# falseywinchnet/PyITD

Hardware: AMD Instinct MI355X
Metric: Msamples/s full ITD (8 levels) + achieved HBM GB/s (higher is better)
Workload: dtype f64

## Files before the change

pyitd_amd/csrc/itd_engine.hip:

```cpp
#include <hip/hip_runtime.h>
#include <hip/hip_ext.h>

#include <algorithm>
#include <cstdio>
#include <cstdlib>
#include <cstring>
#include <type_traits>
#include <atomic>
#include <chrono>
#include <dlfcn.h>
#include <memory>
#include <new>
#include <thread>
#include <vector>

#include "../../include/pyitd_hip.h"
#include "itd_kernels.hpp"
#include "itd_resident.hpp"
#include "itd_knotfirst.hpp"
#include "itd_cubic.hpp"
#include "itd_detect_fast.hpp"
#include "itd_stream.hpp"
#include "itd_tfe.hpp"
#include "itd_tfe_batch.hpp"
// ... 275 lines not shown
    if (tag != ITD_TIME_DECOMPOSE && tag != ITD_TIME_KF_KNOTS) {
        if (e->span_first < 0) e->span_first = k;
        e->span_last = k;
    }
    return k;
}

constexpr int32_t kMaxGridY = 65535;
int chunk_of(const itd_engine *e, int64_t n, int32_t batch)
{
    if (e->chunk > 0) return std::min<int32_t>(std::min<int32_t>(e->chunk, kMaxGridY), batch);
    if ((int64_t)batch * n <= ((int64_t)1 << 24) && batch <= kMaxGridY) return batch;
    const int64_t per = e->batch_streams > 1 ? ((int64_t)1 << 23) : ((int64_t)1 << 24);
    const int64_t c = std::max<int64_t>(1, per / n);
    return (int)std::min<int64_t>(std::min<int64_t>(c, kMaxGridY), batch);
}

inline int64_t seq_samples(const itd_engine *e, int64_t n, int32_t batch) { return (int64_t)std::min<int32_t>(chunk_of(e, n, batch), batch) * n; }

constexpr int kKfLevels = ITD_MAX_ITERATION + 3;
int ensure_kf_ws(itd_engine *e, int tpw, bool may_allocate)
{
    const size_t wgs = (size_t)(e->max_tiles + tpw - 1) / tpw;
    if (e->d_kf && (size_t)e->kf.wgs_max >= wgs) return ITD_OK;
    if (!may_allocate) return ITD_ERR_NOMEM;
    if (e->d_kf) {
        e->kf_retired.push_back(std::move(e->d_kf));
    }
    const size_t B = (size_t)e->max_batch;
    auto al = [](size_t b) { return (b + 255) & ~(size_t)255; };
    const size_t b_sig = al(B * sizeof(KfSig)), b_pool = al(B * wgs * kKcSlab * sizeof(KfEntry));
    const size_t b_first = al(B * kKfLevels * (size_t)e->max_tiles * 4), b_tf = al(B * kKfLevels * (size_t)e->max_tiles * 64);
    const size_t b_tie = al(B * (size_t)e->max_tiles * 64), b_rec = al(B * kKfLevels * wgs * kKcRecGran * 8);
    const size_t total = b_sig + b_pool + b_first + b_tf + b_tie + b_rec;
    const hipError_t rc = e->d_kf.alloc(total, &e->ws_total);
    if (rc != hipSuccess) { fail_hip(e, rc, "hipMalloc(fused levels' workspace)"); return rc == hipErrorOutOfMemory ? ITD_ERR_NOMEM : ITD_ERR_HIP; }
    char *p = (char *)e->d_kf;
    KfWs &w = e->kf;
    w.sig = (KfSig *)p; p += b_sig;
    w.pool = (KfEntry *)p; p += b_pool;
    w.first = (int32_t *)p; p += b_first;
    w.tflags = (unsigned long long *)p; p += b_tf;
    w.nearw = (unsigned long long *)p; p += b_tie;
    w.rec = (unsigned long long *)p;
    if (hipMemset(w.sig, 0, b_sig) != hipSuccess || hipMemset(w.rec, 0, b_rec) != hipSuccess || hipDeviceSynchronize() != hipSuccess) return ITD_ERR_HIP;
    w.wgs_max = (int32_t)wgs; w.rec_levels = kKfLevels;
    {
        int per_cu = 0, cus = 0;
        hipDeviceProp_t prop;
        if (hipOccupancyMaxActiveBlocksPerMultiprocessor(&per_cu, reinterpret_cast<const void *>(&k_kf_knots<T>), kKcThreads, 0) != hipSuccess ||
            hipGetDeviceProperties(&prop, e->device) != hipSuccess) { (void)hipGetLastError(); per_cu = 0; }
        else cus = prop.multiProcessorCount;
        e->kf_resident_wgs = (int64_t)per_cu * cus;
    }
    return ITD_OK;
}

hipError_t launch_timed(itd_engine *e, const void *fn, dim3 grid, dim3 block, void **args, hipStream_t st, int pair)
{
    return hipExtLaunchKernel(fn, grid, block, args, 0, st, pair >= 0 ? e->ev[2 * (size_t)pair] : nullptr,
                              pair >= 0 ? e->ev[2 * (size_t)pair + 1] : nullptr, 0);
}

template <typename Tin>
struct DecomposePlan {
    const Tin *x; int64_t x_stride, n, rows_stride; int32_t M;
    Rows rows; double *bases;
    bool fuse0, nan_input, kf;
    int L0, cap, Mk;
    int n_tiles, n_groups;
    int kf_tpw, kf_wgs;
    SigState *state, *other_state;
    int32_t *gsum, *other_gsum;
    int chunk, S;
};

struct ChunkBufs {
    const itd_engine *e;
    int nb, n_tiles; int64_t n, rows_stride;
    hipStream_t st;
    SigState *state; Rows rows; double *bases, *pp; int32_t *gsum, *counts; TileRec *recs; unsigned long long *near;
    int32_t *gs(int level) const { return gsum + (int64_t)(level % 3) * e->gsum_third; }
    int32_t *cnt(int level) const { return counts + (int64_t)(level & 1) * e->tiles_half; }
    TileRec *rec(int level) const { return recs + (int64_t)(level & 1) * e->tiles_half; }
    double *base(int j) const { return bases ? bases + (int64_t)j * n : pp + (int64_t)(j % 3) * e->pp_pitch; }
    int64_t base_stride() const { return bases ? rows_stride : 3 * e->pp_pitch; }
};

template <typename Trow, typename TIN, bool FIN, int CAPK, int KTW = kTilesPerWave, bool FUSE = false, bool TIES = false>
hipError_t launch_extract(itd_engine *e, const ChunkBufs &c, const TIN *xin, int64_t xs, int j, int pair, int slot)
{
    const TIN *a_x = xin; int64_t a_xs = xs, a_n = c.n, a_rs = c.rows_stride, a_bs = c.base_stride();
    int a_nt = c.n_tiles, a_b = c.nb, a_lvl = j, a_keep = 0;
    const int32_t *a_ci = c.cnt(j), *a_gi = c.gs(j); int32_t *a_co = c.cnt(j + 1), *a_go = c.gs(j + 1), *a_gc = c.gs(j + 2);
    const TileRec *a_ri = c.rec(j); TileRec *a_ro = c.rec(j + 1);
    void *a_rot = c.rows.at((int64_t)std::max(slot, 0) * (c.n + ITD_ROW_PAD)).p; double *a_bas = c.base(j);
    SigState *a_st = c.state; unsigned long long *a_tie = TIES ? c.near : nullptr;
    void *args[] = {&a_x, &a_xs, &a_n, &a_nt, &a_b, &a_ci, &a_co, &a_ri, &a_ro, &a_gi, &a_go, &a_gc, &a_rot, &a_rs,
                    &a_bas, &a_bs, &a_st, &a_lvl, &a_keep, &a_tie};
    const auto launch = [&](auto form) {
        return launch_timed(e, reinterpret_cast<const void *>(&k_extract<TIN, T, FIN, CAPK, KTW, FUSE, TIES, typename decltype(form)::Trow>),
                            dim3((c.n_tiles + KTW - 1) / KTW, c.nb), dim3(kWave), args, c.st, pair);
    };
    return slot < 0 ? launch(RowForm<NoRow, false>{}) : launch(RowForm<Trow, false>{});
}

template <typename Tin>
KfWs kf_chunk_ws(const itd_engine *e, const DecomposePlan<Tin> &p, const int b0, const int nb)
{
    KfWs w = e->kf;
    w.n_tiles = p.n_tiles; w.L0 = p.L0; w.nlev = p.Mk + 3 - p.L0;
    w.cap = p.cap;
    w.xnext = p.cap ? e->d_pp + (int64_t)b0 * 3 * e->pp_pitch + (int64_t)((p.cap - 1) % 3) * e->pp_pitch : nullptr; w.xnext_stride = 3 * e->pp_pitch;
    w.tpw = p.kf_tpw; w.wgs = p.kf_wgs; w.nb = nb;
    w.ticketed = e->policy.tickets((int64_t)w.wgs * nb * p.S, e->kf_resident_wgs) ? 1 : 0;
    w.dbg_kind = e->fault_kind; w.dbg_lev = e->fault_level; w.dbg_wg = e->fault_where; w.dbg_slot = e->fault_slot; w.dbg_delta = e->fault_delta;
    w.dbg_sig = e->fault_sig - b0;
    const size_t B0 = (size_t)b0;
    w.sig += B0; w.pool += B0 * (size_t)w.wgs_max * kKcSlab; w.rec += B0 * (size_t)w.rec_levels * w.wgs_max * kKcRecGran;
    w.first += B0 * (size_t)w.nlev * p.n_tiles; w.tflags += B0 * (size_t)w.nlev * p.n_tiles * 8; w.nearw += B0 * (size_t)p.n_tiles * 8;
    return w;
}

template <typename Form, typename Tin>
int run_chunk(itd_engine *e, const DecomposePlan<Tin> &p, const int b0, const int nb, const hipStream_t cst)
{
    using Trow = typename Form::Trow;
    constexpr bool SEL = Form::SEL;
    const int64_t n = p.n, pp3 = 3 * e->pp_pitch;
    const ChunkBufs c{e, nb, p.n_tiles, n, p.rows_stride, cst, p.state + b0, p.rows.at((int64_t)b0 * p.rows_stride),
                      p.bases ? p.bases + (int64_t)b0 * p.rows_stride : nullptr, e->d_pp + (int64_t)b0 * pp3,
                      p.gsum + (int64_t)b0 * p.n_groups * kGsumPitch, e->d_counts + (int64_t)b0 * p.n_tiles,
                      e->d_recs + (int64_t)b0 * p.n_tiles, p.kf ? e->kf.nearw + (size_t)b0 * p.n_tiles * 8 : nullptr};
    const Tin *xc = p.x + (int64_t)b0 * p.x_stride;
    double *xm_c = c.pp + 2 * e->pp_pitch;
    const dim3 blk(kWave);
    KfFin fin{c.rows.p, p.rows_stride, c.bases ? c.bases : c.pp, c.base_stride(), c.bases ? n : e->pp_pitch, c.bases ? 0 : 3, nullptr,
              p.other_state + b0, p.other_gsum + (int64_t)b0 * p.n_groups * kGsumPitch, e->gsum_third, c.rows.which.res};
    auto levels = [&](const int ja, const int jb) -> int {
        for (int j = ja; j <= jb; ++j) {
            const bool final_level = j == p.M + 1;
            const int pair = time_slot(e, final_level ? ITD_TIME_EXTRACT_FINAL : (j == 0 ? ITD_TIME_EXTRACT_L0 : ITD_TIME_EXTRACT));
            const double *in = j ? c.base(j - 1) : nullptr;
            const int64_t is = c.base_stride();
            hipError_t rc;
            const int slot = c.rows.slot(j, final_level);
            if (j == 0) {
                if (p.nan_input) rc = launch_extract<Trow, double, false, kRankCap0>(e, c, xm_c, pp3, 0, pair, slot);
                else if (p.fuse0) rc = launch_extract<Trow, Tin, false, kRankCap0, kFuse0TilesPerWave, true>(e, c, xc, p.x_stride, 0, pair, slot);
                else rc = launch_extract<Trow, Tin, false, kRankCap0>(e, c, xc, p.x_stride, 0, pair, slot);
            } else if (final_level) rc = launch_extract<Trow, double, true, kRankCap>(e, c, in, is, j, pair, slot);
            else if (p.kf && j == p.L0 - 1) rc = launch_extract<Trow, double, false, kRankCap, kTilesPerWave, false, true>(e, c, in, is, j, pair, slot);
            else rc = launch_extract<Trow, double, false, kRankCap>(e, c, in, is, j, pair, slot);
            if (rc != hipSuccess) return fail_hip(e, rc, "hipExtLaunchKernel(k_extract)");
        }
        return ITD_OK;
    };
    auto finalize = [&]() {
        const int fb = (int)std::min<int64_t>(std::max<int64_t>((n + 8 * kFinalizeThreads - 1) / (8 * kFinalizeThreads), 1), 1024);
        const int jf = p.M + 2;
        k_finalize<Trow, SEL><<<dim3(fb, nb), kFinalizeThreads, 0, cst>>>(static_cast<Trow *>(fin.rows), fin.rows_stride, n, fin.bases, fin.bases_stride,
                                                                          fin.bases_row_pitch, fin.bases_rotate, c.gs(jf), p.n_tiles, jf, c.state,
                                                                          fin.other_state, fin.other_gsum, fin.other_third, fin.res_slot);
    };

    if (p.nan_input) {
        k_nan_level0<Tin, T><<<dim3(p.n_tiles, nb), blk, 0, cst>>>(xc, p.x_stride, n, p.n_tiles, xm_c, pp3, c.cnt(0), c.rec(0), c.gs(0), c.state);
    } else if (!p.fuse0) {
        const Tin *a_x = xc; int64_t a_xs = p.x_stride, a_n = n; int a_nt = p.n_tiles;
        int32_t *a_c = c.cnt(0), *a_g = c.gs(0); TileRec *a_r = c.rec(0); SigState *a_st = c.state; int a_lv = 0;
        void *args[] = {&a_x, &a_xs, &a_n, &a_nt, &a_c, &a_r, &a_g, &a_st, &a_lv};
        HIP_TRY(e, launch_timed(e, reinterpret_cast<const void *>(&k_scan0<Tin, T, kScanTilesPerWave>),
                                dim3((p.n_tiles + kScanTilesPerWave - 1) / kScanTilesPerWave, nb), blk, args, cst, time_slot(e, ITD_TIME_SCAN0)));
    }
    if (const int rc = levels(0, p.kf ? p.L0 - 1 : p.M + 1)) return rc;
    if (!p.kf) {
        finalize();
        return ITD_OK;
    }

    const KfWs w = kf_chunk_ws(e, p, b0, nb);
    const double *xl = c.base(p.L0 - 1);
    const int64_t xl_stride = c.base_stride();
    {
        KfWs a_w = w; int64_t a_ls = xl_stride, a_n = n; const double *a_xl = xl; int a_m = p.Mk;
        const int32_t *a_c = c.cnt(p.L0); const TileRec *a_r = c.rec(p.L0); SigState *a_st = c.state;
        KfFin a_f = fin;
        a_f.gsum = c.gs(p.L0);
        void *args[] = {&a_w, &a_f, &a_xl, &a_ls, &a_n, &a_m, &a_c, &a_r, &a_st};
        HIP_TRY(e, launch_timed(e, reinterpret_cast<const void *>(&k_kf_knots<T, Trow, SEL>), dim3((unsigned)w.wgs * (unsigned)nb), dim3(kKcThreads),
                                args, cst, time_slot(e, ITD_TIME_KF_KNOTS)));
    }
    if (e->fault_kind >= 0 && (e->fault_kind <= 5 || e->fault_kind == 8) && e->fault_level >= p.L0 && e->fault_level - p.L0 < w.nlev &&
        e->fault_where >= 0 && e->fault_where < p.n_tiles && e->fault_sig >= b0 && e->fault_sig < b0 + nb)
        k_kf_fault<<<1, 64, 0, cst>>>(w, e->fault_sig - b0, e->fault_kind, e->fault_level - p.L0, e->fault_where, e->fault_slot & 0xffff, e->fault_delta);
    {
        KfWs a_w = w; const double *a_xl = xl; int64_t a_xs = xl_stride, a_n = n, a_rs = p.rows_stride, a_bs = p.rows_stride;
        const TileRec *a_rec = c.rec(p.L0); void *a_rows = c.rows.p; double *a_bases = c.bases;
        RowSel a_sel = c.rows.which;
        void *args[] = {&a_w, &a_xl, &a_xs, &a_n, &a_rec, &a_rows, &a_rs, &a_bases, &a_bs, &a_sel};
        const auto apply_of = [&](auto with_bases) {
            const auto fn = [](auto part) {
                return reinterpret_cast<const void *>(&k_kf_apply<T, kKfCap, decltype(with_bases)::value, decltype(part)::value, Trow, SEL>);
            };
            return p.cap ? fn(std::true_type{}) : fn(std::false_type{});
        };
        const void *apply_fn = apply_of(std::false_type{});
        if constexpr (std::is_same<Trow, double>::value && !SEL) { if (c.bases) apply_fn = apply_of(std::true_type{}); }
        HIP_TRY(e, launch_timed(e, apply_fn, dim3(p.n_tiles + kf_check_blocks(w.wgs), nb), blk, args, cst, time_slot(e, ITD_TIME_KF_APPLY)));
    }
    if (!p.cap) return ITD_OK;

    const int64_t ge = (int64_t)nb * p.n_groups * kGsumPitch;
    k_clear_gsum<<<(int)std::min<int64_t>((ge + 255) / 256, 1024), 256, 0, cst>>>(c.gs(p.cap), c.gs(p.cap + 1), ge);
    k_scan0<double, T, kScanTilesPerWave><<<dim3((p.n_tiles + kScanTilesPerWave - 1) / kScanTilesPerWave, nb), blk, 0, cst>>>(
        c.base(p.cap - 1), c.base_stride(), n, p.n_tiles, c.cnt(p.cap), c.rec(p.cap), c.gs(p.cap), c.state, p.cap);
    if (const int rc = levels(p.cap, p.M + 1)) return rc;
    finalize();
// ... 2195 lines not shown
```

pyitd_amd/csrc/itd_kernels.hpp:

```cpp
#pragma once
#include <hip/hip_runtime.h>
#include <stdint.h>

#include <type_traits>

#pragma clang fp contract(off)

#ifndef ITD_NT
#define ITD_NT 5
#endif
#ifndef ITD_ABL_R
#define ITD_ABL_R 0
#endif
#ifndef ITD_PRIO
#define ITD_PRIO 0
#endif
#ifndef ITD_EARLY_STOP
#define ITD_EARLY_STOP 1
#endif
#ifndef ITD_BS_SWEEP
#define ITD_BS_SWEEP 1
#endif
namespace itd {

// ... 552 lines not shown
            const int gn = g + 1 < NG ? g + 1 : g;
            const ull le_n = __ballot(d0[gn] <= (T)0), ge_n = __ballot(d0[gn] >= (T)0);
            const ull p1 = __ballot(d1[g] > (T)0), n1 = __ballot(d1[g] < (T)0);
            const ull p2 = (~le >> 1) | (g + 1 < NG ? ~le_n << 63 : plast);
            const ull n2 = (~ge >> 1) | (g + 1 < NG ? ~ge_n << 63 : nlast);
            E[g] = (p1 & le) | (n1 & ge);
            O[g] = (p2 & ~p1) | (n2 & ~n1);
            if (g >= 1 && g + 2 <= NG) zacc |= (le & ge) | ~(p1 | n1);
            le = le_n;
            ge = ge_n;
        }
    } else {
        zacc = ~0ull;
        ull p0 = __ballot(d0[0] > (T)0), n0 = __ballot(d0[0] < (T)0);
#pragma unroll
        for (int g = 0; g < NG; ++g) {
            const int gn = g + 1 < NG ? g + 1 : g;
            const ull p0_n = __ballot(d0[gn] > (T)0), n0_n = __ballot(d0[gn] < (T)0);
            const ull le0 = __ballot(d0[g] <= (T)0), ge0 = __ballot(d0[g] >= (T)0);
            const ull p1 = __ballot(d1[g] > (T)0), n1 = __ballot(d1[g] < (T)0);
            const ull le1 = __ballot(d1[g] <= (T)0), ge1 = __ballot(d1[g] >= (T)0);
            const ull p2 = (p0 >> 1) | (g + 1 < NG ? p0_n << 63 : plast);
            const ull n2 = (n0 >> 1) | (g + 1 < NG ? n0_n << 63 : nlast);
            E[g] = (p1 & le0) | (n1 & ge0);
            O[g] = (p2 & le1) | (n2 & ge1);
            p0 = p0_n;
            n0 = n0_n;
        }
    }
    if (zero_inner) *zero_inner = zacc;
}

constexpr double kNearTie = 0x1p-20;
__device__ __forceinline__ bool near_tie(double a, double b)
{
    return __builtin_fabs(a - b) <= kNearTie * __builtin_fmax(__builtin_fabs(a), __builtin_fabs(b));
}

template <int TW, bool COUNT_ONLY = false, bool NEARF = false>
__device__ __forceinline__ int scan_publish(const double (&xr)[TW / 128][2], double x_lo, double x_hi, int64_t s, int nrem,
                                            size_t slot, size_t gsum_index, int32_t *__restrict__ counts_out,
                                            TileRec *__restrict__ recs_out, int32_t *__restrict__ gsum_out,
                                            int32_t *s_rec , int32_t *s_pos ,
                                            int count_hi = 0 ,
                                            unsigned long long *near_words = nullptr )
{
    constexpr int G2 = TW / 128;
    const int lane = lane_id();
    unsigned long long E[G2], O[G2];
    int total = 0;
    int gcount[G2];
    if (ITD_ABL_R & 4096) {
        total = 3;
#pragma unroll
        for (int g = 0; g < G2; ++g) { gcount[g] = 0; E[g] = O[g] = 0; }
    } else {
        double d0[G2], d1[G2];
        unsigned long long nt0[G2], nt1[G2];
#pragma unroll
        for (int g = 0; g < G2; ++g) {
            const double fill = (g == 0) ? x_lo : wave_dpp<0x13C>(0.0, xr[g > 0 ? g - 1 : 0][1]);
            const double left = wave_dpp<0x138>(fill, xr[g][1]);
            nt0[g] = nt1[g] = 0ull;
            d0[g] = xr[g][0] - left;
            d1[g] = xr[g][1] - xr[g][0];
            if constexpr (NEARF) {
                nt0[g] = __ballot(__builtin_fabs(d0[g]) <= kNearTie * __builtin_fmax(__builtin_fabs(left), __builtin_fabs(xr[g][0])));
                nt1[g] = __ballot(__builtin_fabs(d1[g]) <= kNearTie * __builtin_fmax(__builtin_fabs(xr[g][0]), __builtin_fabs(xr[g][1])));
            }
        }
        knot_predicate<double, G2>(d0, d1, x_hi - xr[G2 - 1][1], E, O);
        if constexpr (NEARF) {
            const unsigned long long nlast = __ballot(near_tie(xr[G2 - 1][1], x_hi)) & (1ull << 63);
            unsigned long long mine = 0ull;
#pragma unroll
            for (int g = 0; g < G2; ++g) {
                unsigned long long Es = nt0[g] | nt1[g];
                unsigned long long Os = nt1[g] | (nt0[g] >> 1) | (g + 1 < G2 ? nt0[g + 1 < G2 ? g + 1 : g] << 63 : nlast);
                const int lo = s > 0 ? 0 : 1, hi = nrem - 2;
                Es &= bit_range((lo - 128 * g + 1) >> 1, (hi - 128 * g) >> 1);
                Os &= bit_range((lo - 128 * g) >> 1, (hi - 128 * g - 1) >> 1);
                if (lane == 2 * g) mine = Es;
                if (lane == 2 * g + 1) mine = Os;
            }
            if (lane < 2 * G2 && near_words) near_words[lane] = mine;
        }
        if ((s == 0) || (nrem <= TW + 1)) {
            const int lo = s > 0 ? 0 : 1, hi = nrem - 2;
#pragma unroll
            for (int g = 0; g < G2; ++g) {
                E[g] &= bit_range((lo - 128 * g + 1) >> 1, (hi - 128 * g) >> 1);
                O[g] &= bit_range((lo - 128 * g) >> 1, (hi - 128 * g - 1) >> 1);
            }
        }
#pragma unroll
        for (int g = 0; g < G2; ++g) {
            gcount[g] = __popcll(E[g]) + __popcll(O[g]);
            total += gcount[g];
        }
    }
    if (lane == 0) {
        if (!(ITD_ABL_R & 32)) counts_out[slot] = total;
        if (count_hi)
            atomicAdd(reinterpret_cast<unsigned long long *>(&gsum_out[gsum_index]), ((unsigned long long)(unsigned)count_hi << 32) | (unsigned)total);
        else if (total && !(ITD_ABL_R & 16)) atomicAdd(&gsum_out[gsum_index], total);
    }
    if constexpr (COUNT_ONLY) return total;
    TileRec *lrec = reinterpret_cast<TileRec *>(s_rec);
    if (lane < 5) s_pos[lane] = 0;
    if (lane == 0) lrec->edge[0] = xr[0][0];
    if (lane == 63) lrec->edge[1] = xr[G2 - 1][1];
    if (total > 0) {
        int gbase = 0;
#pragma unroll
        for (int g = 0; g < G2; ++g) {
            if (gcount[g] > 0 && (gbase < 3 || gbase + gcount[g] > total - 2)) {
                const int bE = lane_bit(E[g]), bO = lane_bit(O[g]);
                const int re = mbcnt64(O[g], mbcnt64(E[g], gbase));
                const int ro_ = re + bE;
                const int pe = 128 * g + 2 * lane;
                if (bE) {
                    if (re < 3) { s_pos[re] = pe; lrec->hval[re] = xr[g][0]; }
                    if (re >= total - 2) { s_pos[3 + re - (total - 2)] = pe; lrec->tval[re - (total - 2)] = xr[g][0]; }
                }
                if (bO) {
                    if (ro_ < 3) { s_pos[ro_] = pe + 1; lrec->hval[ro_] = xr[g][1]; }
                    if (ro_ >= total - 2) { s_pos[3 + ro_ - (total - 2)] = pe + 1; lrec->tval[ro_ - (total - 2)] = xr[g][1]; }
                }
            }
            gbase += gcount[g];
        }
        unsigned flo = 0, fhi = 0;
        auto put = [&](auto gc) {
            constexpr int g = decltype(gc)::value;
            if constexpr (g < G2) {
                flo = write_lane<2 * g>(flo, (unsigned)E[g]);
                fhi = write_lane<2 * g>(fhi, (unsigned)(E[g] >> 32));
                flo = write_lane<2 * g + 1>(flo, (unsigned)O[g]);
                fhi = write_lane<2 * g + 1>(fhi, (unsigned)(O[g] >> 32));
            }
// ... 257 lines not shown
{
    for (int64_t i = (int64_t)blockIdx.x * blockDim.x + threadIdx.x; i < elems; i += (int64_t)gridDim.x * blockDim.x) { a[i] = 0; b[i] = 0; }
}


constexpr int kReach = 8;
#ifndef ITD_PROF
#define ITD_PROF 0
#endif
#if ITD_PROF
__device__ unsigned long long *g_prof_buf;
#define PROF_MARK(i)                                                   \
    if constexpr (FUSE0) {                                             \
        const unsigned long long now__ = __builtin_readcyclecounter(); \
        pt##i += now__ - pt_last;                                      \
        pt_last = now__;                                               \
    }
#else
#define PROF_MARK(i)
#endif
template <typename Tin, int TW, bool FINAL, int CAP, int KT, bool FUSE0 = false, bool TIES = false, typename Trow = double>
__global__ __launch_bounds__(kWave) void k_extract(const Tin *__restrict__ xin, int64_t x_stride, int64_t n,
                                                     int n_tiles, int batch,
                                                     const int32_t *__restrict__ counts_in,
                                                     int32_t *__restrict__ counts_out,
                                                     const TileRec *__restrict__ recs_in,
                                                     TileRec *__restrict__ recs_out,
                                                     const int32_t *__restrict__ gsum_in,
                                                     int32_t *__restrict__ gsum_out, int32_t *__restrict__ gsum_clear,
                                                     Trow *__restrict__ rot_out, int64_t rot_stride,
                                                     double *__restrict__ base_out, int64_t base_stride,
                                                     SigState *__restrict__ state, int level,
                                                     int keep_nan = 0 ,
                                                     unsigned long long *__restrict__ near_out = nullptr )
{
    constexpr int G2 = TW / 128;
    static_assert(TW % 128 == 0 && 2 * G2 <= kMaxGroups, "tile geometry");
    static_assert(CAP >= 128, "a pass must be able to take one 128-sample group");
    static_assert(!FUSE0 || !FINAL, "the fused level-0 launch is never the last level");
    constexpr int RK = CAP + 8;
    __shared__ double s_X[RK];
    __shared__ double s_B[RK];
    __shared__ double s_S[RK];
    __shared__ __attribute__((aligned(16))) int32_t s_rec[sizeof(TileRec) / 4];
    __shared__ double s_bl[2];
    __shared__ int32_t s_pos[8];
    __shared__ __attribute__((aligned(16))) int32_t s_rb[9][16];
    __shared__ double s_hX[8];
    __shared__ int32_t s_hI[8];
    int32_t *s_gi = reinterpret_cast<int32_t *>(s_S);

    const int sig = blockIdx.y;
#if ITD_PROF
    unsigned long long pt_last = __builtin_readcyclecounter(), pt0 = 0, pt1 = 0, pt2 = 0, pt3 = 0, pt4 = 0, pt5 = 0, pt6 = 0, pt7 = 0, pt8 = 0;
    const unsigned long long pt_begin = pt_last;
    const unsigned long long pt_rt0 = __builtin_amdgcn_s_memrealtime();
#endif
    SigState *st = state + sig;
    const Tin *x = xin + (int64_t)sig * x_stride;
    const size_t slot0 = (size_t)sig * n_tiles;
    const int32_t *cnts = counts_in + slot0;
    const TileRec *recs = recs_in + slot0;
    const int n_groups = groups_of(n_tiles);
    const int32_t *gs = gsum_in + (size_t)sig * n_groups * kGsumPitch;
#if ITD_EARLY_STOP
    if constexpr (!FUSE0) {
        const int sl = st->stop_level;
// ... 548 lines not shown
                if (__builtin_expect(__any(nonfinite(be) || nonfinite(bo)), 0)) {
                    odd_vals = true;
                    own_nan = own_nan || __any(__builtin_isunordered(be, bo));
                    if (!keep_nan) {
                        se = be != be ? inf : be;
                        so = bo != bo ? inf : bo;
                    }
                }
                if constexpr (!FINAL) tile_store2<(ITD_NT & 2) != 0>(r_bas, p * 8, se, so);
                if (!FINAL && (near_end || t == 0) && !(ITD_ABL_R & 16384)) {
                    if (t == 0 && p == 0) { ends_next[0] = se; ends_next[1] = so; }
                    if (p == nrem - 2) { ends_next[2] = se; ends_next[3] = so; }
                    if (p + 1 == nrem - 2) ends_next[2] = so;
                    if (p == nrem - 1) ends_next[3] = se;
                }
            }
        }
        rb += m;
        g0 = g1;
        wave_sync();
        PROF_MARK(6)
    }
    if (!(ITD_ABL_R & 65536)) {
        double x_lo = s_bl[0], x_hi = s_bl[1];
        if (__builtin_expect(odd_vals || __any(nonfinite(x_lo) || nonfinite(x_hi)), 0)) {
            const int delta = nan_rules<TW>(xr, x_lo, x_hi, s, nrem);
            if (lane == 0) {
                if (delta) atomicAdd(&st->c_delta[level], delta);
                if (own_nan) atomicOr(&st->nan_mask, 1 << level);
            }
        }
        scan_publish<TW, FINAL, TIES && !FUSE0>(xr, x_lo, x_hi, s, nrem, slot0 + t, ((size_t)sig * n_groups + t / kTilesPerGroup) * kGsumPitch,
                                                counts_out, recs_out, gsum_out, s_rec, s_pos, FUSE0 ? own_c : 0,
                                                (TIES && !FUSE0) ? near_out + (slot0 + t) * 8 : nullptr);
    }
    wave_sync();
    PROF_MARK(7)
  }
    if (blockIdx.x == 0 && !(ITD_ABL_R & 16384)) {
        const int lane = lane_id();
        int acc = 0;
        for (int q = lane; q < n_groups; q += kWave) acc += gs[(size_t)q * kGsumPitch];
#pragma unroll
        for (int d = 32; d >= 1; d >>= 1) acc += __shfl_xor(acc, d);
        int32_t *gc = gsum_clear + (size_t)sig * n_groups * kGsumPitch;
        if (level == 1) {
            int a0 = 0;
            for (int q = lane; q < n_groups; q += kWave) a0 += gs[(size_t)q * kGsumPitch + 1];
#pragma unroll
            for (int d = 32; d >= 1; d >>= 1) a0 += __shfl_xor(a0, d);
            if (lane == 0 && st->m[0] < 0) st->m[0] = a0;
        }
        if (lane == 0 && !FUSE0) {
            if (level >= 1 && ((st->nan_mask >> (level - 1)) & 1)) acc += st->c_delta[level - 1];
            st->m[level] = acc;
            if (level >= 1 && acc < 2 && st->stop_level < 0) st->stop_level = level;
        }
        for (int q = lane; q < n_groups; q += kWave) gc[(size_t)q * kGsumPitch] = 0;
    }
#if ITD_PROF
    if constexpr (FUSE0) {
        PROF_MARK(8)
        if (lane_id() == 0 && g_prof_buf) {
            unsigned long long *o = g_prof_buf + ((size_t)blockIdx.y * gridDim.x + blockIdx.x) * 16;
            o[0] = pt0; o[1] = pt1; o[2] = pt2; o[3] = pt3; o[4] = pt4; o[5] = pt5; o[6] = pt6; o[7] = pt7; o[8] = pt8;
            o[9] = pt_last - pt_begin; o[10] = pt_begin; o[11] = pt_last;
            unsigned xcc; asm volatile("s_getreg_b32 %0, hwreg(HW_REG_XCC_ID)" : "=s"(xcc));
// ... 126 lines not shown
```

pyitd_amd/csrc/itd_knotfirst.hpp:

```cpp
#pragma once
#include "itd_kernels.hpp"

#pragma clang fp contract(off)

namespace itd {

constexpr int kKfCap = 128;

#ifndef ITD_KC_THREADS
#define ITD_KC_THREADS 512
#endif
constexpr int kKcThreads = ITD_KC_THREADS;
constexpr int kKcWaves = kKcThreads / 64;
constexpr int kKcTiles = 64;
constexpr int kKcCap = 1024;
constexpr int kKcCapH = 1720;
constexpr int kKcEnt = (kKcCap + kKcThreads - 1) / kKcThreads;
constexpr int kKcEntH = (kKcCapH + kKcThreads - 1) / kKcThreads;
constexpr int kKcRound = 2;
constexpr int kKcSlab = 3200;
template <bool H>
struct KcLay {
    static constexpr int cap = H ? kKcCapH : kKcCap;
    static constexpr int o_xl = 0, o_xc = 8 * kKcCap, o_xr = 16 * kKcCap;
    static constexpr int o_kX = H ? 0 : 24 * kKcCap;
    static constexpr int o_kB = o_kX + 8 * (cap + 8), o_kS = o_kB + 8 * (cap + 8), o_kpos = o_kS + 8 * (cap + 8);
    static constexpr int o_cpos = o_kpos + 4 * (cap + 8), o_crk = o_cpos + 4 * cap, o_cfl = o_crk + 2 * cap;
    static constexpr int end = o_cfl + cap;
    unsigned char *base;
    __device__ __forceinline__ double *c_xl() const { return reinterpret_cast<double *>(base + o_xl); }
    __device__ __forceinline__ double *c_xc() const { return reinterpret_cast<double *>(base + o_xc); }
    __device__ __forceinline__ double *c_xr() const { return reinterpret_cast<double *>(base + o_xr); }
    __device__ __forceinline__ double *k_X() const { return reinterpret_cast<double *>(base + o_kX); }
    __device__ __forceinline__ double *k_B() const { return reinterpret_cast<double *>(base + o_kB); }
    __device__ __forceinline__ double *k_S() const { return reinterpret_cast<double *>(base + o_kS); }
    __device__ __forceinline__ int32_t *k_pos() const { return reinterpret_cast<int32_t *>(base + o_kpos); }
    __device__ __forceinline__ int32_t *c_pos() const { return reinterpret_cast<int32_t *>(base + o_cpos); }
    __device__ __forceinline__ unsigned short *c_rk() const { return reinterpret_cast<unsigned short *>(base + o_crk); }
    __device__ __forceinline__ unsigned char *c_fl() const { return base + o_cfl; }
};
constexpr int kKcLds = ((KcLay<true>::end > KcLay<false>::end ? KcLay<true>::end : KcLay<false>::end) + 15) & ~15;
static_assert(KcLay<true>::o_kB - KcLay<true>::o_kX >= kKcTiles * 8 * 8, "the sticky words fit the hand-over layout's k_B");
constexpr int kKcRecGran = 32;
constexpr uint32_t kKcPoison = 0xffffffffu;
#ifndef ITD_ROW_PAD
#define ITD_ROW_PAD 0
#endif
#ifndef ITD_KC_GATHER_ORDER
#define ITD_KC_GATHER_ORDER 1
#endif
#ifndef ITD_KF_CHECK_STEP
#define ITD_KF_CHECK_STEP 2
#endif
#ifndef ITD_KC_TIMEOUT
#define ITD_KC_TIMEOUT 4000000ll
#endif

struct KfEntry { double X, B, S; int32_t pos; int32_t pad; };
static_assert(sizeof(KfEntry) == 32, "table entries are two 16-byte words");

constexpr int kKfFailVerify = 1, kKfFailCapacity = 2, kKfFailNonFinite = 4, kKfFailTies = 8;
constexpr int kKfFailWait = 16;

struct KfSig {
    int32_t fail;
    int32_t active;
    int32_t lend;
    int32_t natural;
    int32_t m_exact;
    int32_t fail_lev;
    int32_t cont;
    int32_t pad0[1];
    int32_t mlev[kMaxLevels + 2];
    int32_t acc_mlev[kMaxLevels + 2];
    int32_t acc_fail;
    int32_t nf;
    int32_t done;
    int32_t ticket;
    int32_t fin;
    int32_t pad1;
    uint32_t seq;
    uint32_t pad2;
};
constexpr size_t kKfSigHead = (8 + (kMaxLevels + 2)) * sizeof(int32_t);
static_assert(offsetof(KfSig, acc_mlev) == kKfSigHead, "KfSig layout");
// ... 1 lines not shown
__host__ __device__ inline void kf_sig_verdict(const KfSig &ks, int L0, SigState &st)
{
    if (!ks.active) {
        if (ks.fail) st.kf_fail = ks.fail;
        return;
    }
    int fail = ks.fail;
    const int lend = ks.lend;
    if (lend < 0) fail |= kKfFailCapacity;
    if (!fail && (ks.natural ? ks.m_exact >= 2 : ks.m_exact < 2)) fail |= kKfFailVerify;
    for (int j = L0; !fail && j <= lend; ++j) if (j > L0 && ks.mlev[j] < 2) fail |= kKfFailVerify;
    if (fail) { st.kf_fail = fail; return; }
    for (int j = L0 + 1; j <= lend; ++j) st.m[j] = ks.mlev[j];
    if (ks.cont) return;
    st.m[lend + 1] = ks.m_exact;
    st.fin_stopped = ks.natural;
    st.fin_stop_level = ks.natural ? lend + 1 : -1;
}

struct KfFin {
    void *rows; int64_t rows_stride;
    const double *bases; int64_t bases_stride, bases_row_pitch; int32_t bases_rotate;
    const int32_t *gsum;
    SigState *other_state; int32_t *other_gsum; int64_t other_third;
    int32_t res_slot;
};

struct KfWs {
    KfSig *sig;
    KfEntry *pool;
    int32_t *first;
    unsigned long long *tflags;
    unsigned long long *nearw;
    unsigned long long *rec;
    int32_t wgs_max, rec_levels;
    int32_t nlev, n_tiles, L0;
    int32_t wgs, nb;
    int32_t tpw;
    int32_t ticketed;
    int32_t dbg_kind, dbg_lev, dbg_wg, dbg_slot, dbg_delta;
    int32_t dbg_sig;
    int32_t cap;
    double *xnext; int64_t xnext_stride;
};

__device__ __forceinline__ bool kf_pred(double yl, double yc, double yr)
{
    const double dp = yc - yl, dn = yr - yc;
    return ((dn > 0.0) && (dp <= 0.0)) || ((dn < 0.0) && (dp >= 0.0));
}

__device__ __forceinline__ void kc_store(unsigned long long *p, uint32_t data, uint32_t tag)
{
    __hip_atomic_store(p, ((unsigned long long)tag << 32) | data, __ATOMIC_RELAXED, __HIP_MEMORY_SCOPE_AGENT);
}
__device__ __forceinline__ unsigned long long kc_load(const unsigned long long *p)
{
    return __hip_atomic_load(p, __ATOMIC_RELAXED, __HIP_MEMORY_SCOPE_AGENT);
}
__device__ __forceinline__ void kc_barrier()
{
    asm volatile("s_waitcnt lgkmcnt(0)" ::: "memory");
    __builtin_amdgcn_s_barrier();
    asm volatile("" ::: "memory");
}

// ... 66 lines not shown
    KC_MARK(0);
    int id = blockIdx.x;
    if (ws.ticketed) {
        if (tid == 0) s_i[0] = atomicAdd(&ws.sig[0].ticket, 1);
        kc_barrier();
        id = s_i[0];
    }
    KC_MARK(1);
    const int W = ws.wgs;
    const int sig = id / W, w = id - sig * W;
    if (sig >= ws.nb) return;
    KfSig *ks = ws.sig + sig;
    SigState *st = state + sig;
    const int n_tiles = ws.n_tiles, L0 = ws.L0, M = max_iteration;
    const int tpw = ws.tpw;
    const int t0 = w * tpw, t1 = min(n_tiles, t0 + tpw), nt = t1 - t0;
    const int32_t n1 = (int32_t)(n - 1);
    auto launch_done = [&]() {
        if (ws.ticketed && tid == 192 && atomicAdd(&ws.sig[0].fin, 1) == W * ws.nb - 1) { ws.sig[0].ticket = 0; ws.sig[0].fin = 0; }
    };
    unsigned long long w_in[2], s_in[2];
    int c_in[2];
#pragma unroll
    for (int r = 0; r < 2; ++r) {
        const int q = tid + r * HT, t = t0 + (q >> 3);
        w_in[r] = s_in[r] = 0ull; c_in[r] = 0;
        if (tid < HT && t < t1) {
            c_in[r] = counts[(size_t)sig * n_tiles + t];
            w_in[r] = recs[(size_t)sig * n_tiles + t].flags[q & 7];
            s_in[r] = ws.nearw[((size_t)sig * n_tiles + t) * 8 + (q & 7)];
        }
    }
    const int n_groups = groups_of(n_tiles);
    int m_part = 0;
    {
        const int32_t *gs = fin.gsum + (size_t)sig * n_groups * kGsumPitch;
        for (int g = tid; g < n_groups; g += NT) m_part += gs[(size_t)g * kGsumPitch];
    }
    const double end_in = st->ends[L0 & 1][tid & 3];
    const uint32_t seq = ks->seq;
    int stop_level = st->stop_level;
    const int nan_mask = st->nan_mask, c_delta = L0 >= 1 ? st->c_delta[L0 - 1] : 0;
    const bool odd_input = nan_mask != 0 || st->in_nan || st->l0_fail;
#pragma unroll
    for (int d = 32; d >= 1; d >>= 1) m_part += __shfl_xor(m_part, d);
    if (lane == 0) s_red[wave] = m_part;
    if (tid == 0) s_i[1] = 0;
    kc_barrier();
    bool stopped = stop_level >= 0;
    if (!stopped) {
        int m_last = 0;
#pragma unroll
        for (int k = 0; k < kKcWaves; ++k) m_last += s_red[k];
        if (L0 >= 1 && ((nan_mask >> (L0 - 1)) & 1)) m_last += c_delta;
        if (m_last < 2) { stopped = true; stop_level = L0; }
        if (w == 0 && tid == 0) st->m[L0] = m_last;
    }
    if (w == 0) {
        if (tid == 0) { st->fin_stopped = stopped ? 1 : 0; st->fin_stop_level = stop_level; }
        if (fin.other_state) {
            if (tid == 0) sig_state_reset(fin.other_state + sig);
            int32_t *og = fin.other_gsum + (size_t)sig * n_groups * kGsumPitch;
            for (int k = tid; k < 3 * n_groups; k += NT) {
                int32_t *slot = og + (size_t)(k / n_groups) * fin.other_third + (size_t)(k % n_groups) * kGsumPitch;
                slot[0] = 0;
                slot[1] = 0;
            }
        }
    }
    if (stopped) {
        const int c_row = stop_level - 1;
        Trow *dst = static_cast<Trow *>(fin.rows) + (int64_t)sig * fin.rows_stride + (int64_t)(SEL ? max(fin.res_slot, 0) : c_row) * n;
        const double *src = nullptr;
        if (c_row >= 1) {
            const int row = fin.bases_rotate ? ((c_row - 1) % fin.bases_rotate) : (c_row - 1);
            src = fin.bases + (int64_t)sig * fin.bases_stride + (int64_t)row * fin.bases_row_pitch;
        }
        const int64_t lo = (int64_t)t0 * TW, hi = min((int64_t)t1 * TW, n);
        if (!SEL || fin.res_slot >= 0)
            for (int64_t i = lo + tid; i < hi; i += NT) dst[i] = src ? (Trow)src[i] : (Trow)0.0;
    }
    if (stopped || odd_input) {
        if (w == 0 && tid == 0) {
            ks->active = 0;
            ks->lend = -1;
            ks->fail = stopped ? 0 : kKfFailNonFinite;
            ks->fail_lev = 99;
            ks->cont = 0;
            if (ws.cap && stopped) st->skip = 1;
        }
        launch_done();
        return;
    }
    unsigned long long *rec_sig = ws.rec + ((size_t)sig * ws.rec_levels) * ws.wgs_max * kKcRecGran;
    KfEntry *slab = ws.pool + ((size_t)sig * ws.wgs_max + w) * kKcSlab;
    const int slab_off = w * kKcSlab;
    int32_t *first_sig = ws.first + (size_t)sig * ws.nlev * n_tiles;
    unsigned long long *tf_sig = ws.tflags + (size_t)sig * ws.nlev * n_tiles * 8;
    const double *xs = xl + (int64_t)sig * xl_stride;
    auto rec_slot = [&](int lev, int v) { return rec_sig + ((size_t)(lev - L0) * ws.wgs_max + v) * kKcRecGran; };
    auto rec_tag = [&](int lev) { return seq * 64u + (uint32_t)(lev - L0 + 1); };
    auto give_up = [&](int code) { s_i[1] = 1; atomicOr(&ks->acc_fail, code); };

    unsigned long long *s_w = reinterpret_cast<unsigned long long *>(LH.k_B());
#pragma unroll
    for (int r = 0; r < 2; ++r) {
        const int q = tid + r * HT;
        if (tid < HT) {
            t_w[q] = c_in[r] > 0 ? w_in[r] : 0ull;
            s_w[q] = s_in[r];
        }
    }
    if (tid < 4) s_ends[tid] = end_in;
    if (w == 0 && tid == 0) ks->active = 1;
    kc_barrier();
    KC_MARK(2);
    if (tid == 0) {
        const int64_t p = n - 2;
        const int tp = (int)(p / TW);
        if (p >= 1 && tp >= t0 && tp < t1) {
            const int q = (int)(p - (int64_t)tp * TW);
            s_w[(tp - t0) * 8 + 2 * (q >> 7) + (q & 1)] |= 1ull << ((q & 127) >> 1);
        }
    }
    kc_barrier();
    int c = 0, ck = 0;
    {
        const int tt = (tid >> 2) & (kKcTiles - 1), g = tid & 3;
        const bool mine = tid < HT;
        const unsigned long long Ek = mine ? t_w[tt * 8 + 2 * g] : 0ull, Ok = mine ? t_w[tt * 8 + 2 * g + 1] : 0ull;
        const unsigned long long Es = mine ? s_w[tt * 8 + 2 * g] : 0ull, Os = mine ? s_w[tt * 8 + 2 * g + 1] : 0ull;
        unsigned long long E = Ek | Es, O = Ok | Os;
        int tot;
        int o = kc_scan((__popcll(E) + __popcll(O)) | ((__popcll(Ek) + __popcll(Ok)) << 16), s_red, tot);
        c = tot & 0xffff; ck = tot >> 16;
        int r = o >> 16;
        o &= 0xffff;
        if (c <= kKcCapH) {
            int32_t *c_pos = LH.c_pos(), *k_pos = LH.k_pos();
            unsigned char *c_fl = LH.c_fl();
            unsigned short *c_rk = LH.c_rk();
            const int32_t s = (int32_t)((t0 + tt) * TW + 128 * g);
            while (E | O) {
                const int l = __builtin_ctzll(E | O);
                const unsigned long long bit = 1ull << l;
                if (E & bit) {
                    const int kf = (Ek & bit) ? 1 : 0;
                    r += kf;
                    c_pos[o] = s + 2 * l; c_fl[o] = (unsigned char)(kf | ((Es & bit) ? 2 : 0)); c_rk[o] = (unsigned short)r;
                    if (kf) k_pos[r + 1] = s + 2 * l;
                    ++o;
                }
                if (O & bit) {
                    const int kf = (Ok & bit) ? 1 : 0;
                    r += kf;
                    c_pos[o] = s + 2 * l + 1; c_fl[o] = (unsigned char)(kf | ((Os & bit) ? 2 : 0)); c_rk[o] = (unsigned short)r;
                    if (kf) k_pos[r + 1] = s + 2 * l + 1;
                    ++o;
                }
                E &= ~bit; O &= ~bit;
            }
        } else if (tid == 0) give_up(kKfFailCapacity);
    }
    kc_barrier();
    double va[kKcEntH], vb[kKcEntH], vd[kKcEntH];
#pragma unroll
    for (int i = 0; i < kKcEntH; ++i) va[i] = vb[i] = vd[i] = 0.0;
    if (!s_i[1] && c > 0) {
        int32_t pp[kKcEntH];
#pragma unroll
        for (int i = 0; i < kKcEntH; ++i) pp[i] = LH.c_pos()[min(i * NT + tid, c - 1)];
#if ITD_KC_GATHER_ORDER
#pragma unroll
        for (int i = 0; i < kKcEntH; ++i) vb[i] = xs[pp[i]];
#pragma unroll
        for (int i = 0; i < kKcEntH; ++i) { va[i] = xs[pp[i] - 1]; vd[i] = xs[pp[i] + 1]; }
#else
#pragma unroll
        for (int i = 0; i < kKcEntH; ++i) { va[i] = xs[pp[i] - 1]; vb[i] = xs[pp[i]]; vd[i] = xs[pp[i] + 1]; }
#endif
#pragma unroll
        for (int i = 0; i < kKcEntH; ++i) {
            const int j = i * NT + tid;
            if (j < c && (LH.c_fl()[j] & 1)) LH.k_X()[LH.c_rk()[j] + 1] = vb[i];
        }
        if (tid == 192) atomicAdd(&ks->acc_mlev[L0], ck);
    }
    kc_barrier();
    KC_MARK(3);

    int toff = 0;
    int published = L0 - 1;
    auto level = [&](auto lay, const int lev) -> bool {
        using Lay = decltype(lay);
        constexpr bool FIRST = Lay::cap == kKcCapH;
        constexpr int ENT = FIRST ? kKcEntH : kKcEnt;
        double *const k_X = lay.k_X(), *const k_B = lay.k_B(), *const k_S = lay.k_S();
        int32_t *const k_pos = lay.k_pos();
        const int32_t *const c_pos = lay.c_pos();
        const unsigned short *const c_rk = lay.c_rk();
        const unsigned char *const c_fl = lay.c_fl();
        const int li = lev - L0;
        if (toff + ck + 2 > kKcSlab) { if (tid == 0) give_up(kKfFailCapacity); kc_barrier(); return false; }
        KC_MARK(4 + 4 * min(li, 12));
        if (wave == 2) {
            if (lev == L0) {
                const bool head = w == 0, tail = w == W - 1;
                kc_publish(rec_slot(lev, w), rec_tag(lev), lane, ck, k_pos, k_X, head ? s_ends[0] : (tail ? s_ends[2] : 0.0),
                           head ? s_ends[1] : (tail ? s_ends[3] : 0.0), false);
            }
        } else if (wave == 3) {
            int cnt = 0;
// ... 260 lines not shown
                const int o = (base[i] & 0xffff) + pk[i];
                const int r = (base[i] >> 16) + pn[i] + (nfl[i] & 1);
                if (more && (nfl[i] & 1)) {
                    if (r <= 3) publish_knot(4 + 3 * r, pos[i], yc[i]);
                    if (r == ckn - 1) publish_knot(1, pos[i], yc[i]);
                    if (r == ckn) publish_knot(4, pos[i], yc[i]);
                }
                LN.c_pos()[o] = pos[i]; LN.c_xl()[o] = yl[i]; LN.c_xc()[o] = yc[i]; LN.c_xr()[o] = yr[i]; LN.c_fl()[o] = (unsigned char)nfl[i]; LN.c_rk()[o] = (unsigned short)r;
                if (nfl[i] & 1) {
                    LN.k_pos()[r + 1] = pos[i];
                    LN.k_X()[r + 1] = yc[i];
                    const int tt = pos[i] / TW - t0, q = pos[i] & (TW - 1);
                    atomicOr(&t_w[tt * 8 + 2 * (q >> 7) + (q & 1)], 1ull << ((q & 127) >> 1));
                }
            }
        }
        if (li == 1) KC_MARK(48);
        if (tid == 192) {
            atomicAdd(&ks->acc_mlev[lev + 1], ckn);
            if (w == 0) { s_ends[0] = ne0; s_ends[1] = ne1; }
            if (w == W - 1) { s_ends[2] = ne2; s_ends[3] = 0.0; }
        }
        toff += ck + 2;
        c = tot & 0xffff;
        ck = ckn;
        if (more) published = lev + 1;
        kc_barrier();
        KC_MARK(7 + 4 * min(li, 12));
        return true;
    };
    if (!s_i[1] && level(LH, L0))
        for (int lev = L0 + 1; lev <= M + 1; ++lev)
            if (!level(LN, lev)) break;
    if (s_i[1] && wave == 0) {
        for (int lev = published + 1; lev <= M + 1; ++lev) kc_publish(rec_slot(lev, w), rec_tag(lev), lane, 0, LN.k_pos(), LN.k_X(), 0.0, 0.0, true);
    }
    asm volatile("s_waitcnt vmcnt(0)" ::: "memory");
    kc_barrier();
    if (tid == 192) {
        if (atomicAdd(&ks->done, 1) == W - 1) {
            int lend = M + 1, natural = 0;
            for (int lev = L0; lev <= M + 1; ++lev) {
                if (__hip_atomic_load(&ks->acc_mlev[lev + 1], __ATOMIC_RELAXED, __HIP_MEMORY_SCOPE_AGENT) < 2) { lend = lev; natural = 1; break; }
            }
            const int nf = __hip_atomic_load(&ks->nf, __ATOMIC_RELAXED, __HIP_MEMORY_SCOPE_AGENT);
            int fail = __hip_atomic_load(&ks->acc_fail, __ATOMIC_RELAXED, __HIP_MEMORY_SCOPE_AGENT);
            if (nf && 64 - nf <= lend) fail |= kKfFailNonFinite;
            for (int j = 0; j < kMaxLevels + 2; ++j) {
                ks->mlev[j] = __hip_atomic_load(&ks->acc_mlev[j], __ATOMIC_RELAXED, __HIP_MEMORY_SCOPE_AGENT);
                ks->acc_mlev[j] = 0;
            }
            ks->fail = fail;
            ks->m_exact = 0;
            ks->natural = natural;
            ks->lend = lend;
            ks->fail_lev = nf ? 64 - nf : 99;
            ks->cont = (ws.cap && !natural) ? 1 : 0;
            if (ws.cap && natural) st->skip = 1;
            ks->acc_fail = 0;
            ks->nf = 0;
            ks->done = 0;
            ks->seq = seq + 1;
        }
    }
    launch_done();
#if ITD_PROF
// ... 324 lines not shown
```

Baseline: 44660.

## Stage candidate neighbor triples at scan time and skip the full gsum sweep

The extract scan can now write each tile's first few extremum candidates, with their left and right neighbors, into a compact per-tile buffer. The knot-first kernel then gathers these triples instead of scattering reads into the signal. This path is compiled out by default because ITD_KC_CAND defaults to 0. Separately, the knot kernel stops sweeping every group's gsum up front. It uses the local tile counts and falls back to the full sweep only when the local count is below 2 or the input is odd, with one wave later writing the level total to state. This removes a global reduction from the critical path, at the cost of extra LDS layout and more branches.

```diff
diff --git a/pyitd_amd/csrc/itd_engine.hip b/pyitd_amd/csrc/itd_engine.hip
--- a/pyitd_amd/csrc/itd_engine.hip
+++ b/pyitd_amd/csrc/itd_engine.hip
@@ -331,7 +331,8 @@
     const size_t b_sig = al(B * sizeof(KfSig)), b_pool = al(B * wgs * kKcSlab * sizeof(KfEntry));
     const size_t b_first = al(B * kKfLevels * (size_t)e->max_tiles * 4), b_tf = al(B * kKfLevels * (size_t)e->max_tiles * 64);
     const size_t b_tie = al(B * (size_t)e->max_tiles * 64), b_rec = al(B * kKfLevels * wgs * kKcRecGran * 8);
-    const size_t total = b_sig + b_pool + b_first + b_tf + b_tie + b_rec;
+    const size_t b_cand = al(B * (size_t)e->max_tiles * kCandPitch * 3 * sizeof(double));
+    const size_t total = b_sig + b_pool + b_first + b_tf + b_tie + b_rec + b_cand;
     const hipError_t rc = e->d_kf.alloc(total, &e->ws_total);
     if (rc != hipSuccess) { fail_hip(e, rc, "hipMalloc(fused levels' workspace)"); return rc == hipErrorOutOfMemory ? ITD_ERR_NOMEM : ITD_ERR_HIP; }
     char *p = (char *)e->d_kf;
@@ -341,7 +342,8 @@
     w.first = (int32_t *)p; p += b_first;
     w.tflags = (unsigned long long *)p; p += b_tf;
     w.nearw = (unsigned long long *)p; p += b_tie;
-    w.rec = (unsigned long long *)p;
+    w.rec = (unsigned long long *)p; p += b_rec;
+    w.cand = kCandPitch > 0 ? (double *)p : nullptr;
     if (hipMemset(w.sig, 0, b_sig) != hipSuccess || hipMemset(w.rec, 0, b_rec) != hipSuccess || hipDeviceSynchronize() != hipSuccess) return ITD_ERR_HIP;
     w.wgs_max = (int32_t)wgs; w.rec_levels = kKfLevels;
     {
@@ -378,7 +380,7 @@
     const itd_engine *e;
     int nb, n_tiles; int64_t n, rows_stride;
     hipStream_t st;
-    SigState *state; Rows rows; double *bases, *pp; int32_t *gsum, *counts; TileRec *recs; unsigned long long *near;
+    SigState *state; Rows rows; double *bases, *pp; int32_t *gsum, *counts; TileRec *recs; unsigned long long *near; double *cand;
     int32_t *gs(int level) const { return gsum + (int64_t)(level % 3) * e->gsum_third; }
     int32_t *cnt(int level) const { return counts + (int64_t)(level & 1) * e->tiles_half; }
     TileRec *rec(int level) const { return recs + (int64_t)(level & 1) * e->tiles_half; }
@@ -394,9 +396,9 @@
     const int32_t *a_ci = c.cnt(j), *a_gi = c.gs(j); int32_t *a_co = c.cnt(j + 1), *a_go = c.gs(j + 1), *a_gc = c.gs(j + 2);
     const TileRec *a_ri = c.rec(j); TileRec *a_ro = c.rec(j + 1);
     void *a_rot = c.rows.at((int64_t)std::max(slot, 0) * (c.n + ITD_ROW_PAD)).p; double *a_bas = c.base(j);
-    SigState *a_st = c.state; unsigned long long *a_tie = TIES ? c.near : nullptr;
+    SigState *a_st = c.state; unsigned long long *a_tie = TIES ? c.near : nullptr; double *a_cand = TIES ? c.cand : nullptr;
     void *args[] = {&a_x, &a_xs, &a_n, &a_nt, &a_b, &a_ci, &a_co, &a_ri, &a_ro, &a_gi, &a_go, &a_gc, &a_rot, &a_rs,
-                    &a_bas, &a_bs, &a_st, &a_lvl, &a_keep, &a_tie};
+                    &a_bas, &a_bs, &a_st, &a_lvl, &a_keep, &a_tie, &a_cand};
     const auto launch = [&](auto form) {
         return launch_timed(e, reinterpret_cast<const void *>(&k_extract<TIN, T, FIN, CAPK, KTW, FUSE, TIES, typename decltype(form)::Trow>),
                             dim3((c.n_tiles + KTW - 1) / KTW, c.nb), dim3(kWave), args, c.st, pair);
@@ -418,6 +420,7 @@
     const size_t B0 = (size_t)b0;
     w.sig += B0; w.pool += B0 * (size_t)w.wgs_max * kKcSlab; w.rec += B0 * (size_t)w.rec_levels * w.wgs_max * kKcRecGran;
     w.first += B0 * (size_t)w.nlev * p.n_tiles; w.tflags += B0 * (size_t)w.nlev * p.n_tiles * 8; w.nearw += B0 * (size_t)p.n_tiles * 8;
+    if (w.cand) w.cand += B0 * (size_t)p.n_tiles * kCandPitch * 3;
     return w;
 }
 
@@ -430,7 +433,8 @@
     const ChunkBufs c{e, nb, p.n_tiles, n, p.rows_stride, cst, p.state + b0, p.rows.at((int64_t)b0 * p.rows_stride),
                       p.bases ? p.bases + (int64_t)b0 * p.rows_stride : nullptr, e->d_pp + (int64_t)b0 * pp3,
                       p.gsum + (int64_t)b0 * p.n_groups * kGsumPitch, e->d_counts + (int64_t)b0 * p.n_tiles,
-                      e->d_recs + (int64_t)b0 * p.n_tiles, p.kf ? e->kf.nearw + (size_t)b0 * p.n_tiles * 8 : nullptr};
+                      e->d_recs + (int64_t)b0 * p.n_tiles, p.kf ? e->kf.nearw + (size_t)b0 * p.n_tiles * 8 : nullptr,
+                      p.kf && !p.cap && e->kf.cand ? e->kf.cand + (size_t)b0 * p.n_tiles * kCandPitch * 3 : nullptr};
     const Tin *xc = p.x + (int64_t)b0 * p.x_stride;
     double *xm_c = c.pp + 2 * e->pp_pitch;
     const dim3 blk(kWave);
@@ -483,6 +487,7 @@
     const int64_t xl_stride = c.base_stride();
     {
         KfWs a_w = w; int64_t a_ls = xl_stride, a_n = n; const double *a_xl = xl; int a_m = p.Mk;
+        if (p.cap) a_w.cand = nullptr;
         const int32_t *a_c = c.cnt(p.L0); const TileRec *a_r = c.rec(p.L0); SigState *a_st = c.state;
         KfFin a_f = fin;
         a_f.gsum = c.gs(p.L0);
diff --git a/pyitd_amd/csrc/itd_kernels.hpp b/pyitd_amd/csrc/itd_kernels.hpp
--- a/pyitd_amd/csrc/itd_kernels.hpp
+++ b/pyitd_amd/csrc/itd_kernels.hpp
@@ -608,6 +608,10 @@
 }
 
 constexpr double kNearTie = 0x1p-20;
+#ifndef ITD_KC_CAND
+#define ITD_KC_CAND 0
+#endif
+constexpr int kCandPitch = ITD_KC_CAND;
 __device__ __forceinline__ bool near_tie(double a, double b)
 {
     return __builtin_fabs(a - b) <= kNearTie * __builtin_fmax(__builtin_fabs(a), __builtin_fabs(b));
@@ -619,17 +623,19 @@
                                             TileRec *__restrict__ recs_out, int32_t *__restrict__ gsum_out,
                                             int32_t *s_rec , int32_t *s_pos ,
                                             int count_hi = 0 ,
-                                            unsigned long long *near_words = nullptr )
+                                            unsigned long long *near_words = nullptr ,
+                                            double *cand = nullptr )
 {
     constexpr int G2 = TW / 128;
     const int lane = lane_id();
     unsigned long long E[G2], O[G2];
     int total = 0;
     int gcount[G2];
+    unsigned long long nE[NEARF ? G2 : 1], nO[NEARF ? G2 : 1];
     if (ITD_ABL_R & 4096) {
         total = 3;
 #pragma unroll
-        for (int g = 0; g < G2; ++g) { gcount[g] = 0; E[g] = O[g] = 0; }
+        for (int g = 0; g < G2; ++g) { gcount[g] = 0; E[g] = O[g] = 0; if constexpr (NEARF) nE[g] = nO[g] = 0; }
     } else {
         double d0[G2], d1[G2];
         unsigned long long nt0[G2], nt1[G2];
@@ -658,6 +664,7 @@
                 Os &= bit_range((lo - 128 * g) >> 1, (hi - 128 * g - 1) >> 1);
                 if (lane == 2 * g) mine = Es;
                 if (lane == 2 * g + 1) mine = Os;
+                nE[g] = Es; nO[g] = Os;
             }
             if (lane < 2 * G2 && near_words) near_words[lane] = mine;
         }
@@ -682,6 +689,26 @@
         else if (total && !(ITD_ABL_R & 16)) atomicAdd(&gsum_out[gsum_index], total);
     }
     if constexpr (COUNT_ONLY) return total;
+    if constexpr (NEARF && kCandPitch > 0) {
+        if (cand) {
+            int cbase = 0;
+#pragma unroll
+            for (int g = 0; g < G2; ++g) {
+                const unsigned long long CE = E[g] | nE[g], CO = O[g] | nO[g];
+                if ((CE | CO) && cbase < kCandPitch) {
+                    const double fl = (g == 0) ? x_lo : wave_dpp<0x13C>(0.0, xr[g > 0 ? g - 1 : 0][1]);
+                    const double left = wave_dpp<0x138>(fl, xr[g][1]);
+                    const double fr = (g == G2 - 1) ? x_hi : wave_dpp<0x134>(0.0, xr[g < G2 - 1 ? g + 1 : g][0]);
+                    const double right = wave_dpp<0x130>(fr, xr[g][0]);
+                    const int bE = lane_bit(CE), bO = lane_bit(CO);
+                    const int re = mbcnt64(CO, mbcnt64(CE, cbase)), ro_ = re + bE;
+                    if (bE && re < kCandPitch) { double *c3 = cand + 3 * re; c3[0] = left; c3[1] = xr[g][0]; c3[2] = xr[g][1]; }
+                    if (bO && ro_ < kCandPitch) { double *c3 = cand + 3 * ro_; c3[0] = xr[g][0]; c3[1] = xr[g][1]; c3[2] = right; }
+                }
+                cbase += __popcll(CE) + __popcll(CO);
+            }
+        }
+    }
     TileRec *lrec = reinterpret_cast<TileRec *>(s_rec);
     if (lane < 5) s_pos[lane] = 0;
     if (lane == 0) lrec->edge[0] = xr[0][0];
@@ -1005,7 +1032,8 @@
                                                      double *__restrict__ base_out, int64_t base_stride,
                                                      SigState *__restrict__ state, int level,
                                                      int keep_nan = 0 ,
-                                                     unsigned long long *__restrict__ near_out = nullptr )
+                                                     unsigned long long *__restrict__ near_out = nullptr ,
+                                                     double *__restrict__ cand_out = nullptr )
 {
     constexpr int G2 = TW / 128;
     static_assert(TW % 128 == 0 && 2 * G2 <= kMaxGroups, "tile geometry");
@@ -1620,7 +1648,8 @@
         }
         scan_publish<TW, FINAL, TIES && !FUSE0>(xr, x_lo, x_hi, s, nrem, slot0 + t, ((size_t)sig * n_groups + t / kTilesPerGroup) * kGsumPitch,
                                                 counts_out, recs_out, gsum_out, s_rec, s_pos, FUSE0 ? own_c : 0,
-                                                (TIES && !FUSE0) ? near_out + (slot0 + t) * 8 : nullptr);
+                                                (TIES && !FUSE0) ? near_out + (slot0 + t) * 8 : nullptr,
+                                                (TIES && !FUSE0 && cand_out) ? cand_out + (slot0 + t) * (size_t)(3 * kCandPitch) : nullptr);
     }
     wave_sync();
     PROF_MARK(7)
diff --git a/pyitd_amd/csrc/itd_knotfirst.hpp b/pyitd_amd/csrc/itd_knotfirst.hpp
--- a/pyitd_amd/csrc/itd_knotfirst.hpp
+++ b/pyitd_amd/csrc/itd_knotfirst.hpp
@@ -41,6 +41,7 @@
 };
 constexpr int kKcLds = ((KcLay<true>::end > KcLay<false>::end ? KcLay<true>::end : KcLay<false>::end) + 15) & ~15;
 static_assert(KcLay<true>::o_kB - KcLay<true>::o_kX >= kKcTiles * 8 * 8, "the sticky words fit the hand-over layout's k_B");
+static_assert(kKcLds - KcLay<true>::end >= 2 * kKcTiles && KcLay<true>::end % 2 == 0, "the tiles' first candidates fit behind the hand-over layout");
 constexpr int kKcRecGran = 32;
 constexpr uint32_t kKcPoison = 0xffffffffu;
 #ifndef ITD_ROW_PAD
@@ -51,6 +52,9 @@
 #endif
 #ifndef ITD_KF_CHECK_STEP
 #define ITD_KF_CHECK_STEP 2
+#endif
+#ifndef ITD_KC_SWEEP_ALL
+#define ITD_KC_SWEEP_ALL 0
 #endif
 #ifndef ITD_KC_TIMEOUT
 #define ITD_KC_TIMEOUT 4000000ll
@@ -118,6 +122,7 @@
     int32_t *first;
     unsigned long long *tflags;
     unsigned long long *nearw;
+    double *cand;
     unsigned long long *rec;
     int32_t wgs_max, rec_levels;
     int32_t nlev, n_tiles, L0;
@@ -250,11 +255,13 @@
         }
     }
     const int n_groups = groups_of(n_tiles);
+    const int32_t *const gs = fin.gsum + (size_t)sig * n_groups * kGsumPitch;
     int m_part = 0;
-    {
-        const int32_t *gs = fin.gsum + (size_t)sig * n_groups * kGsumPitch;
-        for (int g = tid; g < n_groups; g += NT) m_part += gs[(size_t)g * kGsumPitch];
-    }
+#if ITD_KC_SWEEP_ALL
+    for (int g = tid; g < n_groups; g += NT) m_part += gs[(size_t)g * kGsumPitch];
+#else
+    if ((tid & 7) == 0) m_part = c_in[0] + c_in[1];
+#endif
     const double end_in = st->ends[L0 & 1][tid & 3];
     const uint32_t seq = ks->seq;
     int stop_level = st->stop_level;
@@ -266,7 +273,27 @@
     if (tid == 0) s_i[1] = 0;
     kc_barrier();
     bool stopped = stop_level >= 0;
-    if (!stopped) {
+#if !ITD_KC_SWEEP_ALL
+    bool swept = false;
+    {
+        int m_own = 0;
+#pragma unroll
+        for (int k = 0; k < kKcWaves; ++k) m_own += s_red[k];
+        swept = !stopped && (odd_input || m_own < 2);
+        if (swept) {
+            m_part = 0;
+            for (int g = tid; g < n_groups; g += NT) m_part += gs[(size_t)g * kGsumPitch];
+#pragma unroll
+            for (int d = 32; d >= 1; d >>= 1) m_part += __shfl_xor(m_part, d);
+            kc_barrier();
+            if (lane == 0) s_red[wave] = m_part;
+            kc_barrier();
+        }
+    }
+#else
+    constexpr bool swept = true;
+#endif
+    if (!stopped && swept) {
         int m_last = 0;
 #pragma unroll
         for (int k = 0; k < kKcWaves; ++k) m_last += s_red[k];
@@ -321,6 +348,7 @@
     auto give_up = [&](int code) { s_i[1] = 1; atomicOr(&ks->acc_fail, code); };
 
     unsigned long long *s_w = reinterpret_cast<unsigned long long *>(LH.k_B());
+    unsigned short *s_tc = reinterpret_cast<unsigned short *>(s_lds + KcLay<true>::end);
 #pragma unroll
     for (int r = 0; r < 2; ++r) {
         const int q = tid + r * HT;
@@ -354,6 +382,7 @@
         c = tot & 0xffff; ck = tot >> 16;
         int r = o >> 16;
         o &= 0xffff;
+        if (mine && g == 0) s_tc[tt] = (unsigned short)o;
         if (c <= kKcCapH) {
             int32_t *c_pos = LH.c_pos(), *k_pos = LH.k_pos();
             unsigned char *c_fl = LH.c_fl();
@@ -385,17 +414,24 @@
 #pragma unroll
     for (int i = 0; i < kKcEntH; ++i) va[i] = vb[i] = vd[i] = 0.0;
     if (!s_i[1] && c > 0) {
-        int32_t pp[kKcEntH];
-#pragma unroll
-        for (int i = 0; i < kKcEntH; ++i) pp[i] = LH.c_pos()[min(i * NT + tid, c - 1)];
+        const double *pv[kKcEntH];
+        const double *const cand_sig = ws.cand ? ws.cand + (size_t)sig * n_tiles * (3 * kCandPitch) : nullptr;
+#pragma unroll
+        for (int i = 0; i < kKcEntH; ++i) {
+            const int j = min(i * NT + tid, c - 1);
+            const int32_t pos = LH.c_pos()[j];
+            const int tile = pos / TW, rk = j - (int)s_tc[tile - t0];
+            const bool blk = cand_sig != nullptr && rk < kCandPitch && pos != n1 - 1;
+            pv[i] = blk ? cand_sig + ((size_t)tile * kCandPitch + rk) * 3 : xs + (pos - 1);
+        }
 #if ITD_KC_GATHER_ORDER
 #pragma unroll
-        for (int i = 0; i < kKcEntH; ++i) vb[i] = xs[pp[i]];
-#pragma unroll
-        for (int i = 0; i < kKcEntH; ++i) { va[i] = xs[pp[i] - 1]; vd[i] = xs[pp[i] + 1]; }
+        for (int i = 0; i < kKcEntH; ++i) vb[i] = pv[i][1];
+#pragma unroll
+        for (int i = 0; i < kKcEntH; ++i) { va[i] = pv[i][0]; vd[i] = pv[i][2]; }
 #else
 #pragma unroll
-        for (int i = 0; i < kKcEntH; ++i) { va[i] = xs[pp[i] - 1]; vb[i] = xs[pp[i]]; vd[i] = xs[pp[i] + 1]; }
+        for (int i = 0; i < kKcEntH; ++i) { va[i] = pv[i][0]; vb[i] = pv[i][1]; vd[i] = pv[i][2]; }
 #endif
 #pragma unroll
         for (int i = 0; i < kKcEntH; ++i) {
@@ -722,6 +758,13 @@
     if (!s_i[1] && level(LH, L0))
         for (int lev = L0 + 1; lev <= M + 1; ++lev)
             if (!level(LN, lev)) break;
+    if (!swept && w == 0 && wave == 4 % kKcWaves) {
+        int tot = 0;
+        for (int g = lane; g < n_groups; g += 64) tot += gs[(size_t)g * kGsumPitch];
+#pragma unroll
+        for (int d = 32; d >= 1; d >>= 1) tot += __shfl_xor(tot, d);
+        if (lane == 0) st->m[L0] = tot;
+    }
     if (s_i[1] && wave == 0) {
         for (int lev = published + 1; lev <= M + 1; ++lev) kc_publish(rec_slot(lev, w), rec_tag(lev), lane, 0, LN.k_pos(), LN.k_X(), 0.0, 0.0, true);
     }
```

Result: no change. 44540 (-0.3%).
